# ChunLI-666/PointCloudProcessor

Hardware: AMD Instinct MI355X
Metric: Mpoints×frames/sec colorized (higher is better)
Workload: dtype f32/f64

## Files before the change

include/pcp_hip.h:

```cpp
#ifndef PCP_HIP_H
#define PCP_HIP_H

#include <stdint.h>

#ifdef __cplusplus
extern "C" {
#endif

#define PCP_ABI_VERSION 6

#define PCP_OK 0
#define PCP_ERR_INVALID (-1)
#define PCP_ERR_STATE (-2)
#define PCP_ERR_DEVICE (-3)
#define PCP_ERR_NOMEM (-4)
#define PCP_ERR_RANGE (-5)

typedef struct pcp_context pcp_context;

typedef struct pcp_pose {
  double x, y, z, qw, qx, qy, qz;
} pcp_pose;

typedef struct pcp_camera {
// ... 356 lines not shown
} pcp_cyl_frame;
int pcp_ortho_begin_cyl(pcp_context *ctx, const pcp_cyl_frame *frame);
int pcp_ortho_cyl_host(const pcp_cyl_frame *frame, int64_t n, const float *xyz, const uint8_t *rgb, const uint8_t *label,
                       const uint8_t *has, int64_t index_base, int32_t fill_radius_px, uint32_t *out_index, float *out_depth,
                       uint8_t *out_rgb, uint8_t *out_label, uint8_t *out_status, int32_t *out_source, int64_t *out_contributors,
                       int64_t *out_occupied, int64_t *out_filled);
int pcp_cyl_angle_host(int64_t n, const double *s, const double *t, double *out_theta);
int pcp_cyl_fit_host(int64_t n, const float *xyz, const float *normal, const uint8_t *has, const double *viewer, float gsd,
                     pcp_cyl_frame *out, double out_stats[8]);
int pcp_ortho_texture_cyl(pcp_context *ctx, const pcp_ortho_texture_params *params, uint8_t *out_rgb, uint8_t *out_mask,
                          uint8_t *out_status, int16_t *out_view, uint8_t *out_count, int64_t out_counts[4]);
int pcp_ortho_texture_points_cyl_host(const pcp_cyl_frame *frame, const pcp_ortho_texture_params *params, const int32_t *source,
                                      const float *depth, float *out_xyz, uint8_t *out_ok);
int pcp_cyl_sincos_host(int64_t n, const double *theta, double *out_sin, double *out_cos);

int pcp_close_pairs(pcp_context *ctx, double radius, int64_t *points_with_close_neighbour);

int pcp_timing_enable(pcp_context *ctx, int32_t on);
int pcp_timing_reset(pcp_context *ctx);
int pcp_timing_get(pcp_context *ctx, int32_t kernel_id, double *total_ms, int64_t *launches);
const char *pcp_kernel_name(int32_t kernel_id);
int pcp_tile_mask_density(pcp_context *ctx, double *kept_fraction);
int pcp_tile_masks(pcp_context *ctx, int64_t *tiles, int32_t *mask_words, uint32_t *out_words);
int pcp_cloud_order(pcp_context *ctx, int32_t *out_perm);
int pcp_tile_bounds(pcp_context *ctx, int64_t *tiles, float *out8);
int pcp_sor_redo_fraction(pcp_context *ctx, double *fraction);
int pcp_sor_distances(pcp_context *ctx, int64_t capacity, float *out_distance);
int pcp_selftest_arithmetic(pcp_context *ctx, int64_t samples, uint64_t seed, int64_t *mismatches_fp64,
                            int64_t *mismatches_fp32);
int pcp_selftest_visit_forms(pcp_context *ctx, int64_t samples, uint64_t seed, int64_t *mismatches_uv, int64_t *mismatches_cell,
                             int64_t *mismatches_sqrt, int32_t *short_distortion);
int pcp_selftest_k3_term(pcp_context *ctx, int64_t samples, uint64_t seed, int64_t *mismatches, int32_t *term_dropped);

#ifdef __cplusplus
}
#endif
#endif
```

pointcloudprocessor_amd/_build.py:

```python
from __future__ import annotations

import os
import subprocess

_PKG = os.path.dirname(os.path.abspath(__file__))
_ROOT = os.path.dirname(_PKG)
CSRC = os.path.join(_PKG, "csrc")
LIB_DIR = os.path.join(_PKG, "lib")
LIB_PATH = os.path.join(LIB_DIR, "libpcp_hip.so")
INCLUDE = os.path.join(_ROOT, "include")

SOURCES = ["pcp_context.hip", "pcp_colour.hip", "pcp_mls.hip", "pcp_grid.hip", "pcp_nid.hip", "pcp_hpr.hip", "pcp_colour_smooth.hip", "pcp_match.hip", "pcp_jpeg.hip",
           "pcp_stream_colour.hip", "pcp_ascii.hip", "pcp_ascii_parse.hip", "pcp_exposure.hip", "pcp_voxel_reduce.hip", "pcp_normals.hip", "pcp_mask_edt.hip", "pcp_ortho.hip", "pcp_ortho_texture.hip", "pcp_facets.hip", "pcp_crack_width.hip", "pcp_crack_fuse.hip", "pcp_crack_length.hip", "pcp_crack_skeleton.hip", "pcp_image_balance.hip"]
HEADERS = ["pcp_internal.hpp", "pcp_device.hpp", "pcp_scan.hpp", "pcp_hsv.hpp", "pcp_exact.hpp", "pcp_ascii.hpp", "pcp_ascii_parse.hpp", "pcp_visit_forms.hpp", "pcp_voxel_reduce.hpp", "pcp_eigen33.hpp", "pcp_eigen33_host.hpp", "pcp_facets.hpp", "pcp_normals.hpp", "pcp_mask_edt.hpp", "pcp_ortho.hpp", "pcp_ortho_cyl.hpp", "pcp_ortho_texture.hpp", "pcp_tile_classify.hpp", "pcp_tile_box.hpp", "pcp_crack_width.hpp", "pcp_crack_fuse.hpp", "pcp_crack_length.hpp", "pcp_crack_skeleton.hpp", "pcp_crack_map.hpp", "pcp_image_balance.hpp"]

HIPCC_FLAGS = [
    "--offload-arch=gfx950",
    "-O3",
    "-std=c++17",
    "-fPIC",
    "-ffp-contract=off",
    "-fhip-fp32-correctly-rounded-divide-sqrt",
    "-Wall",
    "-Wextra",
]


def _hipcc() -> str:
    for cand in (os.environ.get("HIPCC"), "/opt/rocm/bin/hipcc", "hipcc"):
        if cand and (os.path.isabs(cand) and os.path.exists(cand) or not os.path.isabs(cand)):
            return cand
    return "hipcc"


def source_sha256() -> str:
    import hashlib

# ... 57 lines not shown
```

pointcloudprocessor_amd/capi.py:

```python
from __future__ import annotations

import ctypes as C
import os
import re

import numpy as np

from . import _build

PCP_OK = 0
PCP_ERR_INVALID = -1
PCP_ERR_STATE = -2
PCP_ERR_DEVICE = -3
PCP_ERR_NOMEM = -4
PCP_ERR_RANGE = -5

NID_EVAL_FN = C.CFUNCTYPE(C.c_int, C.c_void_p, C.POINTER(C.c_double), C.c_int32, C.POINTER(C.c_double), C.POINTER(C.c_double),
                          C.POINTER(C.c_int32))
K_PROJECT, K_DEPTH, K_COLOUR, K_VISIBILITY, K_MLS_GRID, K_MLS_FIT, K_MISC, K_SOR, K_MLS_VOXEL, K_TILE_MASK, K_NID, K_HPR = range(12)
K_COLOUR_SMOOTH = 12
K_COUNT = 13


class PcpError(RuntimeError):
# ... 1648 lines not shown
    def selftest_arithmetic(self, samples: int = 1 << 26, seed: int = 1):
        a, b = C.c_int64(), C.c_int64()
        self._check(self.lib.pcp_selftest_arithmetic(self.h, C.c_int64(samples), C.c_uint64(seed), C.byref(a), C.byref(b)))
        return a.value, b.value

    def selftest_visit_forms(self, samples: int = 1 << 24, seed: int = 1):
        a, b, c, f = C.c_int64(), C.c_int64(), C.c_int64(), C.c_int32()
        self._check(self.lib.pcp_selftest_visit_forms(self.h, C.c_int64(samples), C.c_uint64(seed), C.byref(a), C.byref(b), C.byref(c),
                                                      C.byref(f)))
        return a.value, b.value, c.value, bool(f.value)

    def selftest_k3_term(self, samples: int = 1 << 24, seed: int = 1):
        a, f = C.c_int64(), C.c_int32()
        self._check(self.lib.pcp_selftest_k3_term(self.h, C.c_int64(samples), C.c_uint64(seed), C.byref(a), C.byref(f)))
        return a.value, bool(f.value)

    def tile_masks(self) -> np.ndarray:
        t, w = C.c_int64(), C.c_int32()
        self._check(self.lib.pcp_tile_masks(self.h, C.byref(t), C.byref(w), None))
        out = np.empty((t.value, w.value), np.uint32)
        self._check(self.lib.pcp_tile_masks(self.h, None, None, _ptr(out)))
        return out

    def cloud_order(self) -> np.ndarray:
        out = np.empty(int(self.lib.pcp_cloud_size(self.h)), np.int32)
        self._check(self.lib.pcp_cloud_order(self.h, _ptr(out)))
        return out

    def tile_bounds(self) -> tuple[np.ndarray, np.ndarray]:
        t = C.c_int64()
        self._check(self.lib.pcp_tile_bounds(self.h, C.byref(t), None))
        groups = (t.value + 15) // 16
        out = np.empty((t.value + groups, 8), np.float32)
        self._check(self.lib.pcp_tile_bounds(self.h, None, _ptr(out)))
        return out[:t.value], out[t.value:]

    def kernel_name(self, kernel_id: int) -> str:
        return self.lib.pcp_kernel_name(C.c_int32(kernel_id)).decode()
```

pointcloudprocessor_amd/csrc/pcp_colour.hip:

```cpp
#include <algorithm>
#include <cfloat>
#include <cstdlib>

#include "pcp_device.hpp"
#include "pcp_hsv.hpp"
#include "pcp_scan.hpp"
#include "pcp_tile_classify.hpp"

namespace pcp {

constexpr int kBlock = 256;
constexpr uint32_t kFltMaxBits = 0x7f7fffffu;

template <bool kCommon>
__device__ __forceinline__ DevCamera common_camera(const DevCamera &in) {
  DevCamera c = in;
  if constexpr (kCommon) {
    c.cull_mode = PCP_CULL_ZBUFFER;
    c.enable_zbuf = 1;
    c.pretest = 1;
    c.ds_fast = 1;
  }
  return c;
}
inline bool is_common_camera(const pcp_context *ctx) {
  const DevCamera &c = ctx->dcam;
  return c.cull_mode == PCP_CULL_ZBUFFER && c.enable_zbuf == 1 && c.pretest == 1 && c.ds_fast == 1 && ctx->uv_tame;
}

struct ProjectOut {
// ... 48 lines not shown
    if (out.pixel) *reinterpret_cast<int4 *>(out.pixel + i0) = pixel;
    if (out.xc) {
      *reinterpret_cast<float4 *>(out.xc + i0) = xc;
      *reinterpret_cast<float4 *>(out.yc + i0) = yc;
      *reinterpret_cast<float4 *>(out.zc + i0) = zc;
    }
  } else {
    for (int64_t i = i0; i < n; ++i) {
      int32_t cell, pixel;
      float range, xc, yc, zc;
      project_store_one(cam, fr, x[i], y[i], z[i], cell, pixel, range, xc, yc, zc);
      if (out.cell) out.cell[i] = cell;
      if (out.range) out.range[i] = range;
      if (out.pixel) out.pixel[i] = pixel;
      if (out.xc) {
        out.xc[i] = xc;
        out.yc[i] = yc;
        out.zc[i] = zc;
      }
    }
  }
}

constexpr int kTileGroup = 16;

__global__ __launch_bounds__(kBlock) void k_group_mask_flat(const float4 *__restrict__ bounds, int64_t groups, DevCamera cam,
                                                            const DevFrame *__restrict__ frames, int32_t n_frames,
                                                            int32_t w0, int32_t w1, int32_t words,
                                                            uint32_t *__restrict__ group_mask,
                                                            uint32_t *__restrict__ group_inside, int32_t cull_enabled,
                                                            int32_t *__restrict__ zeroed, int32_t n_zeroed,
                                                            unsigned long long *__restrict__ far_maps, int64_t far_cells) {
  const int64_t idx = static_cast<int64_t>(blockIdx.x) * kBlock + threadIdx.x;
  if (idx < n_zeroed) zeroed[idx] = 0;
  for (int64_t c = idx; c < far_cells; c += static_cast<int64_t>(gridDim.x) * kBlock) far_maps[c] = 0x7f7f7f7f7f7f7f7full;
  const int32_t nw = w1 - w0;
  const int64_t gw = idx >> 5;
  const int64_t group = gw / nw;
  const bool live = group < groups;
  const int32_t w = w0 + static_cast<int32_t>(gw - group * nw);
  const int32_t f = (w << 5) + static_cast<int32_t>(idx & 31);
  int cls = 1;
  if (live && f < n_frames) cls = cull_enabled ? tile_classify_box(cam, frames[f], bounds[2 * group], bounds[2 * group + 1]) : 0;
  const unsigned long long m = __ballot(cls != 1), in = __ballot(cls == 2);
  if (live && (idx & 31) == 0) {
    group_mask[group * words + w] = static_cast<uint32_t>((threadIdx.x & 32) ? (m >> 32) : m);
    group_inside[group * words + w] = static_cast<uint32_t>((threadIdx.x & 32) ? (in >> 32) : in);
  }
}

template <bool kInside>
__global__ __launch_bounds__(kBlock) void k_tile_mask_dense(const float4 *__restrict__ bounds, int64_t tiles,
                                                            DevCamera cam, const DevFrame *__restrict__ frames,
                                                            int32_t n_frames, int32_t w0, int32_t w1, int32_t words,
                                                            const uint32_t *__restrict__ group_mask,
                                                            const uint32_t *__restrict__ group_inside,
                                                            uint32_t *__restrict__ tile_mask,
                                                            uint32_t *__restrict__ inside_mask, int32_t cull_enabled) {
  const int lane = threadIdx.x & 63;
  const int32_t nw = w1 - w0;
  const int64_t gw = static_cast<int64_t>(blockIdx.x) * (kBlock / 64) + (threadIdx.x >> 6);
  const int64_t group = gw / nw;
  if (group >= (tiles + kTileGroup - 1) / kTileGroup) return;
  const int32_t w = w0 + static_cast<int32_t>(gw - group * nw);
  const int t = lane & 15, slot = lane >> 4;
  const int64_t tile = group * kTileGroup + t;
  const bool have = tile < tiles;
  uint32_t todo = __builtin_amdgcn_readfirstlane(group_mask[group * words + w]);
  const int32_t nb = n_frames - (w << 5);
  if (nb < 32) todo &= nb <= 0 ? 0u : ((1u << nb) - 1u);
// ... 1576 lines not shown
  if (rc != PCP_OK) return rc;
  if (frame_begin < 0 || frame_end > ctx->n_frames || frame_begin > frame_end)
    return set_error(ctx, PCP_ERR_RANGE, "pcp_depth_pass: keyframe range [%d,%d) outside 0..%d", frame_begin, frame_end,
                     ctx->n_frames);
  if (frame_begin == frame_end) return PCP_OK;
  if ((rc = ensure_depth(ctx)) != PCP_OK) return rc;
  const int64_t cells = cells_of(ctx);
  const int64_t map_cells = static_cast<int64_t>(frame_end - frame_begin) * cells;
  const bool z_maps = ctx->n > 0 && ctx->dcam.enable_zbuf;
  if (z_maps) {
    PCP_HIP_TRY(ctx, ctx->depth_sq.ensure(static_cast<size_t>(map_cells) + 4));
  } else if ((rc = fill_u32(ctx, ctx->depth.p + static_cast<int64_t>(frame_begin) * cells, map_cells, kFltMaxBits)) != PCP_OK) {
    return rc;
  }
  if (ctx->n > 0) {
    const size_t plane = plane_of(ctx);
    const int32_t w0 = frame_begin >> 5, w1 = ((frame_end - 1) >> 5) + 1;
    static const bool cull_tiles = [] {
      const char *e = std::getenv("PCP_DISABLE_TILE_CULL");
      return !(e && e[0] == '1');
    }();
    {
      LaunchTimer t(ctx, PCP_K_TILE_MASK);
      const int64_t groups = div_up(ctx->n_tiles, kTileGroup);
      const float4 *tile_bnd = reinterpret_cast<const float4 *>(ctx->tile_bounds.p);
      const size_t gwords = static_cast<size_t>(groups) * ctx->mask_words;
      PCP_HIP_TRY(ctx, ctx->group_mask.ensure(2 * gwords + 8));
      uint32_t *group_inside = ctx->group_mask.p + gwords + 4;
      hipLaunchKernelGGL(k_group_mask_flat, dim3(std::max(blocks_for(groups * (w1 - w0) * 32), blocks_for(2 * kWorkBins))),
                         dim3(kBlock), 0, ctx->stream, tile_bnd + 2 * ctx->n_tiles, groups, ctx->dcam, ctx->frames.p, ctx->n_frames,
                         w0, w1, ctx->mask_words, ctx->group_mask.p, group_inside, cull_tiles ? 1 : 0, ctx->work_hist.p,
                         2 * kWorkBins, z_maps ? reinterpret_cast<unsigned long long *>(ctx->depth_sq.p) : nullptr,
                         z_maps ? map_cells : int64_t(0));
      uint32_t *tile_inside = is_common_camera(ctx) ? nullptr : ctx->tile_inside.p;
      hipLaunchKernelGGL(tile_inside ? k_tile_mask_dense<true> : k_tile_mask_dense<false>, dim3(static_cast<uint32_t>(div_up(groups * (w1 - w0), kBlock / 64))), dim3(kBlock),
                         0, ctx->stream, tile_bnd, ctx->n_tiles, ctx->dcam, ctx->frames.p, ctx->n_frames, w0, w1,
                         ctx->mask_words, ctx->group_mask.p, group_inside, ctx->tile_mask.p, tile_inside, cull_tiles ? 1 : 0);
      if ((rc = sort_tiles_by_work(ctx, w0, w1, ctx->tile_order.p)) != PCP_OK) return rc;
      ctx->tile_order_live = true;
    }
    if (ctx->cull.cull_mode == PCP_CULL_HPR) {
      int rch = ensure_hull_bits(ctx);
      if (rch != PCP_OK) return rch;
      if (!ctx->depth_from_batch) {
        int32_t clear_until = frame_begin;
        for (int32_t f = frame_begin; f < frame_end; ++f) {
          uint32_t *hull_plane = ctx->hull_bits.p + static_cast<size_t>(f >> 5) * static_cast<size_t>(ctx->n);
          if ((f & 31) == 0 && std::min(f + 32, ctx->n_frames) <= frame_end) {
            PCP_HIP_TRY(ctx, hipMemsetAsync(hull_plane, 0, static_cast<size_t>(ctx->n) * 4, ctx->stream));
            clear_until = std::min(f + 32, ctx->n_frames);
          }
          if (f >= clear_until) {
            LaunchTimer t(ctx, PCP_K_HPR);
            hipLaunchKernelGGL(k_hull_clear, dim3(blocks_for(ctx->n)), dim3(kBlock), 0, ctx->stream, hull_plane, ctx->n, 1u << (f & 31));
// ... 388 lines not shown
  std::vector<uint32_t> h(static_cast<size_t>(ctx->n_tiles) * ctx->mask_words);
  PCP_HIP_TRY(ctx, hipMemcpyAsync(h.data(), ctx->tile_mask.p, h.size() * 4, hipMemcpyDeviceToHost, ctx->stream));
  PCP_HIP_TRY(ctx, hipStreamSynchronize(ctx->stream));
  uint64_t bits = 0;
  for (uint32_t w : h) bits += static_cast<uint64_t>(__builtin_popcount(w));
  *kept_fraction = static_cast<double>(bits) / (static_cast<double>(ctx->n_tiles) * ctx->n_frames);
  return PCP_OK;
}

int pcp_tile_masks(pcp_context *ctx, int64_t *tiles, int32_t *mask_words, uint32_t *out_words) {
  if (!ctx) return PCP_ERR_INVALID;
  if (!ctx->tile_mask.p || ctx->n_tiles == 0 || ctx->n_frames == 0)
    return set_error(ctx, PCP_ERR_STATE, "pcp_tile_masks: no masks (call pcp_depth_pass)");
  if (tiles) *tiles = ctx->n_tiles;
  if (mask_words) *mask_words = ctx->mask_words;
  if (out_words) {
    PCP_HIP_TRY(ctx, hipMemcpyAsync(out_words, ctx->tile_mask.p, static_cast<size_t>(ctx->n_tiles) * ctx->mask_words * 4,
                                    hipMemcpyDeviceToHost, ctx->stream));
    PCP_HIP_TRY(ctx, hipStreamSynchronize(ctx->stream));
  }
  return PCP_OK;
}

int pcp_cloud_order(pcp_context *ctx, int32_t *out_perm) {
  if (!ctx || !out_perm) return PCP_ERR_INVALID;
  if (ctx->n == 0) return set_error(ctx, PCP_ERR_STATE, "pcp_cloud_order: no cloud (call pcp_upload_cloud)");
  PCP_HIP_TRY(ctx, hipMemcpyAsync(out_perm, ctx->perm.p, static_cast<size_t>(ctx->n) * 4, hipMemcpyDeviceToHost, ctx->stream));
  PCP_HIP_TRY(ctx, hipStreamSynchronize(ctx->stream));
  return PCP_OK;
}

int pcp_tile_bounds(pcp_context *ctx, int64_t *tiles, float *out8) {
  if (!ctx) return PCP_ERR_INVALID;
  if (ctx->n == 0 || ctx->n_tiles == 0 || !ctx->tile_bounds.p)
    return set_error(ctx, PCP_ERR_STATE, "pcp_tile_bounds: no cloud (call pcp_upload_cloud)");
  if (tiles) *tiles = ctx->n_tiles;
  if (out8) {
    const int64_t groups = div_up(ctx->n_tiles, kTileGroup);
    PCP_HIP_TRY(ctx, hipMemcpyAsync(out8, ctx->tile_bounds.p, static_cast<size_t>(ctx->n_tiles + groups) * 8 * 4, hipMemcpyDeviceToHost,
                                    ctx->stream));
    PCP_HIP_TRY(ctx, hipStreamSynchronize(ctx->stream));
  }
  return PCP_OK;
}

int pcp_colour_result_device(pcp_context *ctx, void **device_ptr, int64_t *n_words) {
// ... 114 lines not shown
```

pointcloudprocessor_amd/csrc/pcp_context.hip:

```cpp
#include <algorithm>
#include <cfloat>
#include <cmath>
#include <cstdlib>
#include <new>
#include <vector>

#include "pcp_internal.hpp"
#include "pcp_crack_map.hpp"
#include "pcp_visit_forms.hpp"
#include "pcp_scan.hpp"

namespace pcp {

static thread_local std::string g_error;

int set_error(const pcp_context *ctx, int code, const char *fmt, ...) {
  char buf[1024];
  va_list ap;
  va_start(ap, fmt);
  vsnprintf(buf, sizeof(buf), fmt, ap);
  va_end(ap);
  if (ctx)
    ctx->error = buf;
  else
    g_error = buf;
  return code;
}

void set_global_error(const char *fmt, ...) {
  char buf[1024];
  va_list ap;
  va_start(ap, fmt);
  vsnprintf(buf, sizeof(buf), fmt, ap);
// ... 254 lines not shown
                                                       int64_t n, float *__restrict__ sx, float *__restrict__ sy,
                                                       float *__restrict__ sz, int32_t *__restrict__ inv_perm) {
  const int64_t j = static_cast<int64_t>(blockIdx.x) * kUpBlock + threadIdx.x;
  if (j >= n) return;
  const int32_t i = perm[j];
  sx[j] = x[i];
  sy[j] = y[i];
  sz[j] = z[i];
  if (inv_perm) inv_perm[i] = static_cast<int32_t>(j);
}

template <int kSpan>
__global__ __launch_bounds__(kUpBlock) void k_up_bounds(const float *__restrict__ sx, const float *__restrict__ sy,
                                                        const float *__restrict__ sz, int64_t n,
                                                        float4 *__restrict__ out, int64_t count) {
  constexpr int kLanes = kSpan >= kUpBlock ? kUpBlock : kSpan;
  constexpr int kPer = kSpan / kLanes;
  constexpr int kSpheresPerBlock = kUpBlock / kLanes;
  __shared__ double red[10][kUpBlock / 64];
  const int sub = threadIdx.x / kLanes, l = threadIdx.x % kLanes;
  const int64_t sphere = static_cast<int64_t>(blockIdx.x) * kSpheresPerBlock + sub;
  const int64_t b = sphere * kSpan;
  double lo[3] = {1e300, 1e300, 1e300}, hi[3] = {-1e300, -1e300, -1e300};
  float px[kPer], py[kPer], pz[kPer];
  bool have[kPer];
#pragma unroll
  for (int q = 0; q < kPer; ++q) {
    const int64_t j = b + static_cast<int64_t>(q) * kLanes + l;
    have[q] = sphere < count && j < n;
    px[q] = have[q] ? sx[j] : 0.0f;
    py[q] = have[q] ? sy[j] : 0.0f;
    pz[q] = have[q] ? sz[j] : 0.0f;
    if (have[q]) {
      lo[0] = fmin(lo[0], static_cast<double>(px[q])); hi[0] = fmax(hi[0], static_cast<double>(px[q]));
      lo[1] = fmin(lo[1], static_cast<double>(py[q])); hi[1] = fmax(hi[1], static_cast<double>(py[q]));
      lo[2] = fmin(lo[2], static_cast<double>(pz[q])); hi[2] = fmax(hi[2], static_cast<double>(pz[q]));
    }
  }
#pragma unroll
  for (int a = 0; a < 3; ++a)
    for (int o = (kLanes < 64 ? kLanes : 64) / 2; o >= 1; o >>= 1) {
      lo[a] = fmin(lo[a], __shfl_xor(lo[a], o, 64));
      hi[a] = fmax(hi[a], __shfl_xor(hi[a], o, 64));
    }
  if (kLanes > 64) {
    if ((threadIdx.x & 63) == 0)
      for (int a = 0; a < 3; ++a) {
        red[a][threadIdx.x >> 6] = lo[a];
        red[3 + a][threadIdx.x >> 6] = hi[a];
      }
    __syncthreads();
    for (int a = 0; a < 3; ++a)
      for (int k = 0; k < kUpBlock / 64; ++k) {
        lo[a] = fmin(lo[a], red[a][k]);
        hi[a] = fmax(hi[a], red[3 + a][k]);
      }
    __syncthreads();
  }
  float c[3];
#pragma unroll
  for (int a = 0; a < 3; ++a) c[a] = static_cast<float>(0.5 * (lo[a] + hi[a]));
  double r2 = 0.0, h[3] = {0.0, 0.0, 0.0};
#pragma unroll
  for (int q = 0; q < kPer; ++q)
    if (have[q]) {
      const double dx = static_cast<double>(px[q]) - static_cast<double>(c[0]);
      const double dy = static_cast<double>(py[q]) - static_cast<double>(c[1]);
      const double dz = static_cast<double>(pz[q]) - static_cast<double>(c[2]);
      r2 = fmax(r2, (dx * dx + dy * dy) + dz * dz);
      h[0] = fmax(h[0], fabs(dx));
      h[1] = fmax(h[1], fabs(dy));
      h[2] = fmax(h[2], fabs(dz));
    }
  for (int o = (kLanes < 64 ? kLanes : 64) / 2; o >= 1; o >>= 1) {
    r2 = fmax(r2, __shfl_xor(r2, o, 64));
#pragma unroll
    for (int a = 0; a < 3; ++a) h[a] = fmax(h[a], __shfl_xor(h[a], o, 64));
  }
  if (kLanes > 64) {
    if ((threadIdx.x & 63) == 0) {
      red[6][threadIdx.x >> 6] = r2;
      for (int a = 0; a < 3; ++a) red[7 + a][threadIdx.x >> 6] = h[a];
    }
    __syncthreads();
    for (int k = 0; k < kUpBlock / 64; ++k) {
      r2 = fmax(r2, red[6][k]);
      for (int a = 0; a < 3; ++a) h[a] = fmax(h[a], red[7 + a][k]);
    }
  }
  if (l == 0 && sphere < count) {
    const auto up = [](double v) {
      const float r = static_cast<float>(v * (1.0 + 1e-6));
      return isfinite(r) ? __uint_as_float(__float_as_uint(r) + 1u) : r;
    };
    out[2 * sphere] = make_float4(c[0], c[1], c[2], up(sqrt(r2)));
    out[2 * sphere + 1] = make_float4(up(h[0]), up(h[1]), up(h[2]), 0.0f);
// ... 117 lines not shown
    hipLaunchKernelGGL(k_up_deinterleave, dim3(up_blocks(n)), dim3(kUpBlock), 0, st, static_cast<const uint32_t *>(aos), stride / 4, n,
                       dx, dy, dz);
  } else if (aos) {
    PCP_HIP_TRY(ctx, raw.ensure(static_cast<size_t>(n) * static_cast<size_t>(stride) / 4 + 4));
    PCP_HIP_TRY(ctx, hipMemcpyAsync(raw.p, aos, static_cast<size_t>(n) * static_cast<size_t>(stride), hipMemcpyHostToDevice, st));
    hipLaunchKernelGGL(k_up_deinterleave, dim3(up_blocks(n)), dim3(kUpBlock), 0, st, raw.p, stride / 4, n, dx, dy, dz);
  } else {
    PCP_HIP_TRY(ctx, hipMemcpyAsync(dx, x, sn * 4, hipMemcpyHostToDevice, st));
    PCP_HIP_TRY(ctx, hipMemcpyAsync(dy, y, sn * 4, hipMemcpyHostToDevice, st));
    PCP_HIP_TRY(ctx, hipMemcpyAsync(dz, z, sn * 4, hipMemcpyHostToDevice, st));
  }
  float mn[3], mx[3];
  unsigned long long nonfinite = 0;
  PCP_HIP_TRY(ctx, ctx->inv_perm.ensure(plane + 4));
  if (int rc = spatial_order(ctx, dx, dy, dz, n, ctx->perm.p, ctx->sxyz.p, ctx->sxyz.p + plane, ctx->sxyz.p + 2 * plane,
                             ctx->inv_perm.p, mn, mx, &nonfinite))
    return rc;
  raw.release();
  ctx->nonfinite_points = static_cast<int64_t>(nonfinite);
  for (int a = 0; a < 3; ++a) {
    ctx->host_min[a] = mn[a];
    ctx->host_max[a] = mx[a];
  }
  const int64_t tiles = (n + 63) / 64, groups = (tiles + 15) / 16;
  PCP_HIP_TRY(ctx, ctx->tile_bounds.ensure(static_cast<size_t>(tiles + groups) * 8 + 4));
  float4 *sph = reinterpret_cast<float4 *>(ctx->tile_bounds.p);
  hipLaunchKernelGGL(k_up_bounds<64>, dim3(static_cast<uint32_t>((tiles + 3) / 4)), dim3(kUpBlock), 0, st, ctx->sxyz.p,
                     ctx->sxyz.p + plane, ctx->sxyz.p + 2 * plane, n, sph, tiles);
  hipLaunchKernelGGL(k_up_bounds<1024>, dim3(static_cast<uint32_t>(groups)), dim3(kUpBlock), 0, st, ctx->sxyz.p,
                     ctx->sxyz.p + plane, ctx->sxyz.p + 2 * plane, n, sph + 2 * tiles, groups);
  PCP_HIP_TRY(ctx, hipGetLastError());
  ctx->n_tiles = tiles;
  PCP_HIP_TRY(ctx, hipStreamSynchronize(st));
  return PCP_OK;
}

}

using namespace pcp;

extern "C" {

int pcp_abi_version(void) { return PCP_ABI_VERSION; }

int pcp_create(int32_t device, pcp_context **out) {
  if (!out) {
    set_global_error("pcp_create: out is NULL");
    return PCP_ERR_INVALID;
  }
  *out = nullptr;
  int count = 0;
  hipError_t e = hipGetDeviceCount(&count);
  if (e != hipSuccess || count <= 0) {
// ... 408 lines not shown
```

pointcloudprocessor_amd/host_build.py:

```python
from __future__ import annotations

import os
import subprocess

from . import _build

HOST = os.path.join(os.path.dirname(os.path.abspath(__file__)), "host")
BIN = os.path.join(HOST, "bin")
ROCM = os.environ.get("ROCM_PATH", "/opt/rocm")

TARGETS = {
    "pcp_shim_selftest": ["shim_selftest.cpp"],
    "PointCloudProcessor": ["main.cpp"],
    "image_dump": ["image_dump.cpp"],
    "format_selftest": ["format_selftest.cpp"],
    "parse_selftest": ["parse_selftest.cpp"],
    "visit_forms_selftest": ["visit_forms_selftest.cpp"],
    "k3_term_selftest": ["k3_term_selftest.cpp"],
    "voxel_reduce_selftest": ["voxel_reduce_selftest.cpp"],
    "normals_selftest": ["normals_selftest.cpp"],
    "ortho_selftest": ["ortho_selftest.cpp"],
    "ortho_texture_selftest": ["ortho_texture_selftest.cpp"],
    "crack_width_selftest": ["crack_width_selftest.cpp"],
    "crack_fuse_selftest": ["crack_fuse_selftest.cpp"],
    "crack_length_selftest": ["crack_length_selftest.cpp"],
    "crack_skeleton_selftest": ["crack_skeleton_selftest.cpp"],
    "image_balance_selftest": ["image_balance_selftest.cpp"],
    "ortho_cyl_selftest": ["ortho_cyl_selftest.cpp"],
    "ortho_cyl_texture_selftest": ["ortho_cyl_texture_selftest.cpp"],
    "facets_selftest": ["facets_selftest.cpp"],
    "tile_bounds_selftest": ["tile_bounds_selftest.cpp"],
}


def build(force: bool = False) -> dict:
    os.makedirs(BIN, exist_ok=True)
    out = {}
    for name, srcs in TARGETS.items():
        exe = os.path.join(BIN, name)
        deps = [os.path.join(HOST, s) for s in srcs] + [os.path.join(HOST, "pcp_shim.hpp"), os.path.join(HOST, "pcp_multi.hpp"), os.path.join(HOST, "pcd_io.hpp"), os.path.join(HOST, "image_io.hpp"), os.path.join(HOST, "pcd_device_reader.hpp"),
                                                       os.path.join(_build.CSRC, "pcp_ascii_parse.hpp"), os.path.join(_build.CSRC, "pcp_ascii.hpp"), os.path.join(_build.CSRC, "pcp_visit_forms.hpp"), os.path.join(_build.CSRC, "pcp_voxel_reduce.hpp"), os.path.join(_build.CSRC, "pcp_normals.hpp"), os.path.join(_build.CSRC, "pcp_ortho.hpp"), os.path.join(_build.CSRC, "pcp_ortho_cyl.hpp"), os.path.join(_build.CSRC, "pcp_ortho_texture.hpp"), os.path.join(_build.CSRC, "pcp_crack_width.hpp"), os.path.join(_build.CSRC, "pcp_crack_fuse.hpp"), os.path.join(_build.CSRC, "pcp_crack_length.hpp"), os.path.join(_build.CSRC, "pcp_crack_skeleton.hpp"), os.path.join(_build.CSRC, "pcp_image_balance.hpp"), os.path.join(_build.CSRC, "pcp_hsv.hpp"), os.path.join(_build.CSRC, "pcp_facets.hpp"), os.path.join(_build.CSRC, "pcp_eigen33_host.hpp"), os.path.join(_build.CSRC, "pcp_tile_box.hpp"),
                                                       os.path.join(_build.INCLUDE, "pcp_hip.h")]
        deps = [d for d in deps if os.path.exists(d)]
        stale = force or not os.path.exists(exe) or any(os.path.getmtime(d) > os.path.getmtime(exe) for d in deps)
        if stale:
            extra = os.environ.get("PCP_HOST_CXXFLAGS", "").split()
            multi = ["-D__HIP_PLATFORM_AMD__", "-isystem", os.path.join(ROCM, "include")] if name == "PointCloudProcessor" else []
            multi_libs = ["-L", os.path.join(ROCM, "lib"), "-lrccl", "-lamdhip64", "-Wl,-rpath," + os.path.join(ROCM, "lib")] \
                if name == "PointCloudProcessor" else []
            cmd = ["g++", "-std=c++17", "-O2", "-ffp-contract=off", "-pthread", "-Wall", "-Wextra"] + extra + multi + ["-I", _build.INCLUDE, "-I", HOST] + [
                os.path.join(HOST, s) for s in srcs] + ["-L", _build.LIB_DIR, "-lpcp_hip"] + multi_libs + [
                                                        "-lz", "-Wl,-rpath,$ORIGIN/../../lib", "-o", exe]
            proc = subprocess.run(cmd, capture_output=True, text=True)
            if proc.returncode != 0:
                raise RuntimeError(f"g++ failed for {name}:\n{proc.stderr[-3000:]}")
        out[name] = exe
    return out
```

Measured before the change: 2.079 million.

## Cull tile groups top-down through a new block level of bounding boxes

Result: no change. 2.078 million (-0.1%).

```diff
diff --git a/include/pcp_hip.h b/include/pcp_hip.h
--- a/include/pcp_hip.h
+++ b/include/pcp_hip.h
@@ -402,6 +402,7 @@
 const char *pcp_kernel_name(int32_t kernel_id);
 int pcp_tile_mask_density(pcp_context *ctx, double *kept_fraction);
 int pcp_tile_masks(pcp_context *ctx, int64_t *tiles, int32_t *mask_words, uint32_t *out_words);
+int pcp_tile_work(pcp_context *ctx, int64_t *tiles, int32_t *out_work);
 int pcp_cloud_order(pcp_context *ctx, int32_t *out_perm);
 int pcp_tile_bounds(pcp_context *ctx, int64_t *tiles, float *out8);
 int pcp_sor_redo_fraction(pcp_context *ctx, double *fraction);
diff --git a/pointcloudprocessor_amd/_build.py b/pointcloudprocessor_amd/_build.py
--- a/pointcloudprocessor_amd/_build.py
+++ b/pointcloudprocessor_amd/_build.py
@@ -12,7 +12,7 @@
 
 SOURCES = ["pcp_context.hip", "pcp_colour.hip", "pcp_mls.hip", "pcp_grid.hip", "pcp_nid.hip", "pcp_hpr.hip", "pcp_colour_smooth.hip", "pcp_match.hip", "pcp_jpeg.hip",
            "pcp_stream_colour.hip", "pcp_ascii.hip", "pcp_ascii_parse.hip", "pcp_exposure.hip", "pcp_voxel_reduce.hip", "pcp_normals.hip", "pcp_mask_edt.hip", "pcp_ortho.hip", "pcp_ortho_texture.hip", "pcp_facets.hip", "pcp_crack_width.hip", "pcp_crack_fuse.hip", "pcp_crack_length.hip", "pcp_crack_skeleton.hip", "pcp_image_balance.hip"]
-HEADERS = ["pcp_internal.hpp", "pcp_device.hpp", "pcp_scan.hpp", "pcp_hsv.hpp", "pcp_exact.hpp", "pcp_ascii.hpp", "pcp_ascii_parse.hpp", "pcp_visit_forms.hpp", "pcp_voxel_reduce.hpp", "pcp_eigen33.hpp", "pcp_eigen33_host.hpp", "pcp_facets.hpp", "pcp_normals.hpp", "pcp_mask_edt.hpp", "pcp_ortho.hpp", "pcp_ortho_cyl.hpp", "pcp_ortho_texture.hpp", "pcp_tile_classify.hpp", "pcp_tile_box.hpp", "pcp_crack_width.hpp", "pcp_crack_fuse.hpp", "pcp_crack_length.hpp", "pcp_crack_skeleton.hpp", "pcp_crack_map.hpp", "pcp_image_balance.hpp"]
+HEADERS = ["pcp_internal.hpp", "pcp_device.hpp", "pcp_scan.hpp", "pcp_hsv.hpp", "pcp_exact.hpp", "pcp_ascii.hpp", "pcp_ascii_parse.hpp", "pcp_visit_forms.hpp", "pcp_voxel_reduce.hpp", "pcp_eigen33.hpp", "pcp_eigen33_host.hpp", "pcp_facets.hpp", "pcp_normals.hpp", "pcp_mask_edt.hpp", "pcp_ortho.hpp", "pcp_ortho_cyl.hpp", "pcp_ortho_texture.hpp", "pcp_tile_classify.hpp", "pcp_tile_box.hpp", "pcp_tile_levels.hpp", "pcp_crack_width.hpp", "pcp_crack_fuse.hpp", "pcp_crack_length.hpp", "pcp_crack_skeleton.hpp", "pcp_crack_map.hpp", "pcp_image_balance.hpp"]
 
 HIPCC_FLAGS = [
     "--offload-arch=gfx950",
diff --git a/pointcloudprocessor_amd/capi.py b/pointcloudprocessor_amd/capi.py
--- a/pointcloudprocessor_amd/capi.py
+++ b/pointcloudprocessor_amd/capi.py
@@ -1694,6 +1694,13 @@
         self._check(self.lib.pcp_tile_masks(self.h, None, None, _ptr(out)))
         return out
 
+    def tile_work(self) -> np.ndarray:
+        t = C.c_int64()
+        self._check(self.lib.pcp_tile_work(self.h, C.byref(t), None))
+        out = np.empty(t.value, np.int32)
+        self._check(self.lib.pcp_tile_work(self.h, None, _ptr(out)))
+        return out
+
     def cloud_order(self) -> np.ndarray:
         out = np.empty(int(self.lib.pcp_cloud_size(self.h)), np.int32)
         self._check(self.lib.pcp_cloud_order(self.h, _ptr(out)))
diff --git a/pointcloudprocessor_amd/csrc/pcp_colour.hip b/pointcloudprocessor_amd/csrc/pcp_colour.hip
--- a/pointcloudprocessor_amd/csrc/pcp_colour.hip
+++ b/pointcloudprocessor_amd/csrc/pcp_colour.hip
@@ -6,6 +6,7 @@
 #include "pcp_hsv.hpp"
 #include "pcp_scan.hpp"
 #include "pcp_tile_classify.hpp"
+#include "pcp_tile_levels.hpp"
 
 namespace pcp {
 
@@ -100,30 +101,59 @@
   }
 }
 
-constexpr int kTileGroup = 16;
-
-__global__ __launch_bounds__(kBlock) void k_group_mask_flat(const float4 *__restrict__ bounds, int64_t groups, DevCamera cam,
-                                                            const DevFrame *__restrict__ frames, int32_t n_frames,
-                                                            int32_t w0, int32_t w1, int32_t words,
-                                                            uint32_t *__restrict__ group_mask,
-                                                            uint32_t *__restrict__ group_inside, int32_t cull_enabled,
-                                                            int32_t *__restrict__ zeroed, int32_t n_zeroed,
-                                                            unsigned long long *__restrict__ far_maps, int64_t far_cells) {
+constexpr int kTileGroup = kGroupTiles;
+
+__global__ __launch_bounds__(kBlock) void k_group_mask_top_down(const float4 *__restrict__ bounds,
+                                                                const float4 *__restrict__ block_bounds, int64_t groups,
+                                                                int64_t blocks, DevCamera cam,
+                                                                const DevFrame *__restrict__ frames, int32_t n_frames,
+                                                                int32_t w0, int32_t w1, int32_t words,
+                                                                uint32_t *__restrict__ group_mask,
+                                                                uint32_t *__restrict__ group_inside, int32_t cull_enabled,
+                                                                int32_t *__restrict__ zeroed, int32_t n_zeroed,
+                                                                unsigned long long *__restrict__ far_maps, int64_t far_cells) {
+  __shared__ uint32_t s_keep[kBlockGroups][kSpanWords], s_in[kBlockGroups][kSpanWords];
+  __shared__ int32_t s_list[64];
+  __shared__ int32_t s_count;
   const int64_t idx = static_cast<int64_t>(blockIdx.x) * kBlock + threadIdx.x;
   if (idx < n_zeroed) zeroed[idx] = 0;
   for (int64_t c = idx; c < far_cells; c += static_cast<int64_t>(gridDim.x) * kBlock) far_maps[c] = 0x7f7f7f7f7f7f7f7full;
-  const int32_t nw = w1 - w0;
-  const int64_t gw = idx >> 5;
-  const int64_t group = gw / nw;
-  const bool live = group < groups;
-  const int32_t w = w0 + static_cast<int32_t>(gw - group * nw);
-  const int32_t f = (w << 5) + static_cast<int32_t>(idx & 31);
-  int cls = 1;
-  if (live && f < n_frames) cls = cull_enabled ? tile_classify_box(cam, frames[f], bounds[2 * group], bounds[2 * group + 1]) : 0;
-  const unsigned long long m = __ballot(cls != 1), in = __ballot(cls == 2);
-  if (live && (idx & 31) == 0) {
-    group_mask[group * words + w] = static_cast<uint32_t>((threadIdx.x & 32) ? (m >> 32) : m);
-    group_inside[group * words + w] = static_cast<uint32_t>((threadIdx.x & 32) ? (in >> 32) : in);
+  const int32_t spans = mask_spans(w0, w1);
+  const int64_t blk = blockIdx.x / spans;
+  if (blk >= blocks) return;
+  const int32_t wb = w0 + (static_cast<int32_t>(blockIdx.x - blk * spans)) * kSpanWords;
+  const int32_t ng = block_group_count(blk, groups);
+  const int64_t g0 = block_first_group(blk);
+  if (threadIdx.x < 64) {
+    const int32_t lane = threadIdx.x;
+    const int32_t f = (wb << 5) + lane;
+    int cls = 1;
+    if (wb + (lane >> 5) < w1 && f < n_frames)
+      cls = cull_enabled ? tile_classify_box(cam, frames[f], block_bounds[2 * blk], block_bounds[2 * blk + 1]) : 0;
+    const unsigned long long in = __ballot(cls == 2), open = __ballot(cls == 0);
+    if (lane < kBlockGroups * kSpanWords)
+      s_keep[lane / kSpanWords][lane % kSpanWords] = s_in[lane / kSpanWords][lane % kSpanWords] =
+          static_cast<uint32_t>(in >> (32 * (lane % kSpanWords)));
+    if (cls == 0) s_list[__popcll(open & ((1ull << lane) - 1ull))] = lane;
+    if (lane == 0) s_count = __popcll(open);
+  }
+  __syncthreads();
+  const int32_t pairs = s_count * kBlockGroups;
+  for (int32_t p = threadIdx.x; p < pairs; p += kBlock) {
+    const int32_t g = p % kBlockGroups, k = s_list[p / kBlockGroups];
+    if (g < ng) {
+      const int cls = cull_enabled ? tile_classify_box(cam, frames[(wb << 5) + k], bounds[2 * (g0 + g)], bounds[2 * (g0 + g) + 1]) : 0;
+      if (cls != 1) atomicOr(&s_keep[g][k >> 5], 1u << (k & 31));
+      if (cls == 2) atomicOr(&s_in[g][k >> 5], 1u << (k & 31));
+    }
+  }
+  __syncthreads();
+  if (threadIdx.x < kBlockGroups * kSpanWords) {
+    const int32_t g = threadIdx.x / kSpanWords, w = wb + threadIdx.x % kSpanWords;
+    if (g < ng && w < w1) {
+      group_mask[(g0 + g) * words + w] = s_keep[g][threadIdx.x % kSpanWords];
+      group_inside[(g0 + g) * words + w] = s_in[g][threadIdx.x % kSpanWords];
+    }
   }
 }
 
@@ -1746,14 +1776,16 @@
     }();
     {
       LaunchTimer t(ctx, PCP_K_TILE_MASK);
-      const int64_t groups = div_up(ctx->n_tiles, kTileGroup);
+      const TileLevels lv = tile_levels(ctx->n);
+      const int64_t groups = lv.groups;
       const float4 *tile_bnd = reinterpret_cast<const float4 *>(ctx->tile_bounds.p);
       const size_t gwords = static_cast<size_t>(groups) * ctx->mask_words;
       PCP_HIP_TRY(ctx, ctx->group_mask.ensure(2 * gwords + 8));
       uint32_t *group_inside = ctx->group_mask.p + gwords + 4;
-      hipLaunchKernelGGL(k_group_mask_flat, dim3(std::max(blocks_for(groups * (w1 - w0) * 32), blocks_for(2 * kWorkBins))),
-                         dim3(kBlock), 0, ctx->stream, tile_bnd + 2 * ctx->n_tiles, groups, ctx->dcam, ctx->frames.p, ctx->n_frames,
-                         w0, w1, ctx->mask_words, ctx->group_mask.p, group_inside, cull_tiles ? 1 : 0, ctx->work_hist.p,
+      hipLaunchKernelGGL(k_group_mask_top_down,
+                         dim3(std::max(static_cast<uint32_t>(lv.blocks * mask_spans(w0, w1)), blocks_for(2 * kWorkBins))), dim3(kBlock), 0,
+                         ctx->stream, tile_bnd + 2 * lv.group_at, tile_bnd + 2 * lv.block_at, groups, lv.blocks, ctx->dcam, ctx->frames.p,
+                         ctx->n_frames, w0, w1, ctx->mask_words, ctx->group_mask.p, group_inside, cull_tiles ? 1 : 0, ctx->work_hist.p,
                          2 * kWorkBins, z_maps ? reinterpret_cast<unsigned long long *>(ctx->depth_sq.p) : nullptr,
                          z_maps ? map_cells : int64_t(0));
       uint32_t *tile_inside = is_common_camera(ctx) ? nullptr : ctx->tile_inside.p;
@@ -2188,6 +2220,18 @@
   return PCP_OK;
 }
 
+int pcp_tile_work(pcp_context *ctx, int64_t *tiles, int32_t *out_work) {
+  if (!ctx) return PCP_ERR_INVALID;
+  if (!ctx->tile_work.p || !ctx->tile_order_live || ctx->n_tiles == 0)
+    return set_error(ctx, PCP_ERR_STATE, "pcp_tile_work: no tile order (call pcp_depth_pass)");
+  if (tiles) *tiles = ctx->n_tiles;
+  if (out_work) {
+    PCP_HIP_TRY(ctx, hipMemcpyAsync(out_work, ctx->tile_work.p, static_cast<size_t>(ctx->n_tiles) * 4, hipMemcpyDeviceToHost, ctx->stream));
+    PCP_HIP_TRY(ctx, hipStreamSynchronize(ctx->stream));
+  }
+  return PCP_OK;
+}
+
 int pcp_cloud_order(pcp_context *ctx, int32_t *out_perm) {
   if (!ctx || !out_perm) return PCP_ERR_INVALID;
   if (ctx->n == 0) return set_error(ctx, PCP_ERR_STATE, "pcp_cloud_order: no cloud (call pcp_upload_cloud)");
diff --git a/pointcloudprocessor_amd/csrc/pcp_context.hip b/pointcloudprocessor_amd/csrc/pcp_context.hip
--- a/pointcloudprocessor_amd/csrc/pcp_context.hip
+++ b/pointcloudprocessor_amd/csrc/pcp_context.hip
@@ -9,6 +9,7 @@
 #include "pcp_crack_map.hpp"
 #include "pcp_visit_forms.hpp"
 #include "pcp_scan.hpp"
+#include "pcp_tile_levels.hpp"
 
 namespace pcp {
 
@@ -309,19 +310,33 @@
   const int64_t sphere = static_cast<int64_t>(blockIdx.x) * kSpheresPerBlock + sub;
   const int64_t b = sphere * kSpan;
   double lo[3] = {1e300, 1e300, 1e300}, hi[3] = {-1e300, -1e300, -1e300};
-  float px[kPer], py[kPer], pz[kPer];
-  bool have[kPer];
+  constexpr bool kKeep = kPer <= 4;
+  constexpr int kKept = kKeep ? kPer : 1;
+  float px[kKept], py[kKept], pz[kKept];
+  bool have[kKept];
+  if constexpr (kKeep) {
 #pragma unroll
-  for (int q = 0; q < kPer; ++q) {
-    const int64_t j = b + static_cast<int64_t>(q) * kLanes + l;
-    have[q] = sphere < count && j < n;
-    px[q] = have[q] ? sx[j] : 0.0f;
-    py[q] = have[q] ? sy[j] : 0.0f;
-    pz[q] = have[q] ? sz[j] : 0.0f;
-    if (have[q]) {
-      lo[0] = fmin(lo[0], static_cast<double>(px[q])); hi[0] = fmax(hi[0], static_cast<double>(px[q]));
-      lo[1] = fmin(lo[1], static_cast<double>(py[q])); hi[1] = fmax(hi[1], static_cast<double>(py[q]));
-      lo[2] = fmin(lo[2], static_cast<double>(pz[q])); hi[2] = fmax(hi[2], static_cast<double>(pz[q]));
+    for (int q = 0; q < kPer; ++q) {
+      const int64_t j = b + static_cast<int64_t>(q) * kLanes + l;
+      have[q] = sphere < count && j < n;
+      px[q] = have[q] ? sx[j] : 0.0f;
+      py[q] = have[q] ? sy[j] : 0.0f;
+      pz[q] = have[q] ? sz[j] : 0.0f;
+      if (have[q]) {
+        lo[0] = fmin(lo[0], static_cast<double>(px[q])); hi[0] = fmax(hi[0], static_cast<double>(px[q]));
+        lo[1] = fmin(lo[1], static_cast<double>(py[q])); hi[1] = fmax(hi[1], static_cast<double>(py[q]));
+        lo[2] = fmin(lo[2], static_cast<double>(pz[q])); hi[2] = fmax(hi[2], static_cast<double>(pz[q]));
+      }
+    }
+  } else {
+    for (int q = 0; q < kPer; ++q) {
+      const int64_t j = b + static_cast<int64_t>(q) * kLanes + l;
+      if (sphere < count && j < n) {
+        const double vx = sx[j], vy = sy[j], vz = sz[j];
+        lo[0] = fmin(lo[0], vx); hi[0] = fmax(hi[0], vx);
+        lo[1] = fmin(lo[1], vy); hi[1] = fmax(hi[1], vy);
+        lo[2] = fmin(lo[2], vz); hi[2] = fmax(hi[2], vz);
+      }
     }
   }
 #pragma unroll
@@ -348,17 +363,25 @@
 #pragma unroll
   for (int a = 0; a < 3; ++a) c[a] = static_cast<float>(0.5 * (lo[a] + hi[a]));
   double r2 = 0.0, h[3] = {0.0, 0.0, 0.0};
+  const auto member = [&](float mx, float my, float mz) {
+    const double dx = static_cast<double>(mx) - static_cast<double>(c[0]);
+    const double dy = static_cast<double>(my) - static_cast<double>(c[1]);
+    const double dz = static_cast<double>(mz) - static_cast<double>(c[2]);
+    r2 = fmax(r2, (dx * dx + dy * dy) + dz * dz);
+    h[0] = fmax(h[0], fabs(dx));
+    h[1] = fmax(h[1], fabs(dy));
+    h[2] = fmax(h[2], fabs(dz));
+  };
+  if constexpr (kKeep) {
 #pragma unroll
-  for (int q = 0; q < kPer; ++q)
-    if (have[q]) {
-      const double dx = static_cast<double>(px[q]) - static_cast<double>(c[0]);
-      const double dy = static_cast<double>(py[q]) - static_cast<double>(c[1]);
-      const double dz = static_cast<double>(pz[q]) - static_cast<double>(c[2]);
-      r2 = fmax(r2, (dx * dx + dy * dy) + dz * dz);
-      h[0] = fmax(h[0], fabs(dx));
-      h[1] = fmax(h[1], fabs(dy));
-      h[2] = fmax(h[2], fabs(dz));
-    }
+    for (int q = 0; q < kPer; ++q)
+      if (have[q]) member(px[q], py[q], pz[q]);
+  } else {
+    for (int q = 0; q < kPer; ++q) {
+      const int64_t j = b + static_cast<int64_t>(q) * kLanes + l;
+      if (sphere < count && j < n) member(sx[j], sy[j], sz[j]);
+    }
+  }
   for (int o = (kLanes < 64 ? kLanes : 64) / 2; o >= 1; o >>= 1) {
     r2 = fmax(r2, __shfl_xor(r2, o, 64));
 #pragma unroll
@@ -522,13 +545,16 @@
     ctx->host_min[a] = mn[a];
     ctx->host_max[a] = mx[a];
   }
-  const int64_t tiles = (n + 63) / 64, groups = (tiles + 15) / 16;
-  PCP_HIP_TRY(ctx, ctx->tile_bounds.ensure(static_cast<size_t>(tiles + groups) * 8 + 4));
+  const TileLevels lv = tile_levels(n);
+  const int64_t tiles = lv.tiles, groups = lv.groups;
+  PCP_HIP_TRY(ctx, ctx->tile_bounds.ensure(static_cast<size_t>(lv.records) * 8 + 4));
   float4 *sph = reinterpret_cast<float4 *>(ctx->tile_bounds.p);
-  hipLaunchKernelGGL(k_up_bounds<64>, dim3(static_cast<uint32_t>((tiles + 3) / 4)), dim3(kUpBlock), 0, st, ctx->sxyz.p,
+  hipLaunchKernelGGL(k_up_bounds<kTilePlaces>, dim3(static_cast<uint32_t>((tiles + 3) / 4)), dim3(kUpBlock), 0, st, ctx->sxyz.p,
                      ctx->sxyz.p + plane, ctx->sxyz.p + 2 * plane, n, sph, tiles);
-  hipLaunchKernelGGL(k_up_bounds<1024>, dim3(static_cast<uint32_t>(groups)), dim3(kUpBlock), 0, st, ctx->sxyz.p,
-                     ctx->sxyz.p + plane, ctx->sxyz.p + 2 * plane, n, sph + 2 * tiles, groups);
+  hipLaunchKernelGGL(k_up_bounds<kGroupPlaces>, dim3(static_cast<uint32_t>(groups)), dim3(kUpBlock), 0, st, ctx->sxyz.p,
+                     ctx->sxyz.p + plane, ctx->sxyz.p + 2 * plane, n, sph + 2 * lv.group_at, groups);
+  hipLaunchKernelGGL(k_up_bounds<kBlockPlaces>, dim3(static_cast<uint32_t>(lv.blocks)), dim3(kUpBlock), 0, st, ctx->sxyz.p,
+                     ctx->sxyz.p + plane, ctx->sxyz.p + 2 * plane, n, sph + 2 * lv.block_at, lv.blocks);
   PCP_HIP_TRY(ctx, hipGetLastError());
   ctx->n_tiles = tiles;
   PCP_HIP_TRY(ctx, hipStreamSynchronize(st));
diff --git a/pointcloudprocessor_amd/csrc/pcp_tile_levels.hpp b/pointcloudprocessor_amd/csrc/pcp_tile_levels.hpp
--- /dev/null
+++ b/pointcloudprocessor_amd/csrc/pcp_tile_levels.hpp
@@ -0,0 +1,46 @@
+#pragma once
+
+#include <cstdint>
+
+#if defined(__HIPCC__)
+#include <hip/hip_runtime.h>
+#define PCP_TL_HD __host__ __device__ __forceinline__
+#else
+#define PCP_TL_HD inline
+#endif
+
+namespace pcp {
+
+constexpr int kTilePlaces = 64;
+constexpr int kGroupTiles = 16;
+constexpr int kBlockGroups = 16;
+constexpr int kGroupPlaces = kTilePlaces * kGroupTiles;
+constexpr int kBlockPlaces = kGroupPlaces * kBlockGroups;
+
+struct TileLevels {
+  int64_t tiles, groups, blocks;
+  int64_t group_at, block_at;
+  int64_t records;
+};
+
+PCP_TL_HD TileLevels tile_levels(int64_t n) {
+  TileLevels t;
+  t.tiles = (n + kTilePlaces - 1) / kTilePlaces;
+  t.groups = (t.tiles + kGroupTiles - 1) / kGroupTiles;
+  t.blocks = (t.groups + kBlockGroups - 1) / kBlockGroups;
+  t.group_at = t.tiles;
+  t.block_at = t.tiles + t.groups;
+  t.records = t.tiles + t.groups + t.blocks;
+  return t;
+}
+
+PCP_TL_HD int64_t block_first_group(int64_t b) { return b * kBlockGroups; }
+PCP_TL_HD int32_t block_group_count(int64_t b, int64_t groups) {
+  const int64_t left = groups - b * kBlockGroups;
+  return static_cast<int32_t>(left < 0 ? 0 : left > kBlockGroups ? kBlockGroups : left);
+}
+
+constexpr int kSpanWords = 2;
+PCP_TL_HD int32_t mask_spans(int32_t w0, int32_t w1) { return (w1 - w0 + kSpanWords - 1) / kSpanWords; }
+
+}
diff --git a/pointcloudprocessor_amd/host/tile_levels_selftest.cpp b/pointcloudprocessor_amd/host/tile_levels_selftest.cpp
--- /dev/null
+++ b/pointcloudprocessor_amd/host/tile_levels_selftest.cpp
@@ -0,0 +1,90 @@
+#include <cstdint>
+#include <cstdio>
+#include <cstdlib>
+#include <vector>
+
+#include "../csrc/pcp_tile_levels.hpp"
+
+static long failures = 0;
+#define CHECK(cond)                                                        \
+  do {                                                                     \
+    if (!(cond)) {                                                         \
+      if (++failures < 20) std::printf("FAILED line %d: %s\n", __LINE__, #cond); \
+    }                                                                      \
+  } while (0)
+
+static std::vector<int32_t> tile_places, group_tiles, block_groups;
+static void add_place(int64_t j) {
+  const size_t t = static_cast<size_t>(j / 64);
+  if (t >= tile_places.size()) {
+    tile_places.push_back(0);
+    const size_t g = t / 16;
+    if (g >= group_tiles.size()) {
+      group_tiles.push_back(0);
+      const size_t b = g / 16;
+      if (b >= block_groups.size()) block_groups.push_back(0);
+      ++block_groups[b];
+    }
+    ++group_tiles[g];
+  }
+  ++tile_places[t];
+}
+static void check_by_walking(int64_t n) {
+  if (n > 0) add_place(n - 1);
+  const pcp::TileLevels lv = pcp::tile_levels(n);
+  CHECK(lv.tiles == static_cast<int64_t>(tile_places.size()));
+  CHECK(lv.groups == static_cast<int64_t>(group_tiles.size()));
+  CHECK(lv.blocks == static_cast<int64_t>(block_groups.size()));
+  CHECK(lv.group_at == lv.tiles && lv.block_at == lv.tiles + lv.groups && lv.records == lv.block_at + lv.blocks);
+  int64_t seen = 0;
+  for (int64_t b = 0; b < lv.blocks; ++b) {
+    CHECK(pcp::block_first_group(b) == seen);
+    CHECK(pcp::block_group_count(b, lv.groups) == block_groups[static_cast<size_t>(b)]);
+    seen += pcp::block_group_count(b, lv.groups);
+  }
+  CHECK(seen == lv.groups);
+  CHECK(pcp::block_group_count(lv.blocks, lv.groups) == 0 && pcp::block_group_count(lv.blocks + 5, lv.groups) == 0);
+}
+
+static void check_large(int64_t n) {
+  const pcp::TileLevels lv = pcp::tile_levels(n);
+  CHECK(lv.tiles * 64 >= n && (lv.tiles - 1) * 64 < n);
+  CHECK(lv.groups * 16 >= lv.tiles && (lv.groups - 1) * 16 < lv.tiles);
+  CHECK(lv.blocks * 16 >= lv.groups && (lv.blocks - 1) * 16 < lv.groups);
+  CHECK(lv.records == lv.tiles + lv.groups + lv.blocks);
+  int64_t seen = 0;
+  for (int64_t b = 0; b < lv.blocks; ++b) {
+    const int32_t c = pcp::block_group_count(b, lv.groups);
+    CHECK(c >= 1 && c <= 16 && (c == 16 || b == lv.blocks - 1));
+    seen += c;
+  }
+  CHECK(seen == lv.groups);
+}
+
+static void check_spans() {
+  for (int32_t w0 = 0; w0 < 70; ++w0)
+    for (int32_t w1 = w0 + 1; w1 < 140; ++w1) {
+      std::vector<int> hit(static_cast<size_t>(w1), 0);
+      const int32_t spans = pcp::mask_spans(w0, w1);
+      for (int32_t s = 0; s < spans; ++s)
+        for (int k = 0; k < pcp::kSpanWords; ++k) {
+          const int32_t w = w0 + s * pcp::kSpanWords + k;
+          if (w < w1) ++hit[static_cast<size_t>(w)];
+        }
+      for (int32_t w = 0; w < w1; ++w) CHECK(hit[static_cast<size_t>(w)] == (w >= w0 ? 1 : 0));
+    }
+}
+
+int main(int argc, char **argv) {
+  const int64_t limit = argc > 1 ? std::atoll(argv[1]) : 70000;
+  static_assert(pcp::kGroupPlaces == 1024 && pcp::kBlockPlaces == 16384, "level spans");
+  for (int64_t n = 0; n <= limit; ++n) check_by_walking(n);
+  const int64_t edges[] = {65535, 65536, 65537, 16384 * 16 - 1, 16384 * 16, 16384 * 16 + 1, 10000000, (int64_t(1) << 31) - 1,
+                           int64_t(1) << 31, (int64_t(1) << 31) + 1, (int64_t(1) << 32) + 12345};
+  for (int64_t n : edges) check_large(n);
+  check_spans();
+  std::printf("tile levels: sizes 0 ... %ld walked, %zu large sizes, word ranges up to 140 words\n", static_cast<long>(limit),
+              sizeof(edges) / sizeof(edges[0]));
+  std::printf("tile_levels_selftest: %ld failures\n", failures);
+  return failures ? 1 : 0;
+}
diff --git a/pointcloudprocessor_amd/host_build.py b/pointcloudprocessor_amd/host_build.py
--- a/pointcloudprocessor_amd/host_build.py
+++ b/pointcloudprocessor_amd/host_build.py
@@ -30,6 +30,7 @@
     "ortho_cyl_texture_selftest": ["ortho_cyl_texture_selftest.cpp"],
     "facets_selftest": ["facets_selftest.cpp"],
     "tile_bounds_selftest": ["tile_bounds_selftest.cpp"],
+    "tile_levels_selftest": ["tile_levels_selftest.cpp"],
 }
 
 
@@ -39,7 +40,7 @@
     for name, srcs in TARGETS.items():
         exe = os.path.join(BIN, name)
         deps = [os.path.join(HOST, s) for s in srcs] + [os.path.join(HOST, "pcp_shim.hpp"), os.path.join(HOST, "pcp_multi.hpp"), os.path.join(HOST, "pcd_io.hpp"), os.path.join(HOST, "image_io.hpp"), os.path.join(HOST, "pcd_device_reader.hpp"),
-                                                       os.path.join(_build.CSRC, "pcp_ascii_parse.hpp"), os.path.join(_build.CSRC, "pcp_ascii.hpp"), os.path.join(_build.CSRC, "pcp_visit_forms.hpp"), os.path.join(_build.CSRC, "pcp_voxel_reduce.hpp"), os.path.join(_build.CSRC, "pcp_normals.hpp"), os.path.join(_build.CSRC, "pcp_ortho.hpp"), os.path.join(_build.CSRC, "pcp_ortho_cyl.hpp"), os.path.join(_build.CSRC, "pcp_ortho_texture.hpp"), os.path.join(_build.CSRC, "pcp_crack_width.hpp"), os.path.join(_build.CSRC, "pcp_crack_fuse.hpp"), os.path.join(_build.CSRC, "pcp_crack_length.hpp"), os.path.join(_build.CSRC, "pcp_crack_skeleton.hpp"), os.path.join(_build.CSRC, "pcp_image_balance.hpp"), os.path.join(_build.CSRC, "pcp_hsv.hpp"), os.path.join(_build.CSRC, "pcp_facets.hpp"), os.path.join(_build.CSRC, "pcp_eigen33_host.hpp"), os.path.join(_build.CSRC, "pcp_tile_box.hpp"),
+                                                       os.path.join(_build.CSRC, "pcp_ascii_parse.hpp"), os.path.join(_build.CSRC, "pcp_ascii.hpp"), os.path.join(_build.CSRC, "pcp_visit_forms.hpp"), os.path.join(_build.CSRC, "pcp_voxel_reduce.hpp"), os.path.join(_build.CSRC, "pcp_normals.hpp"), os.path.join(_build.CSRC, "pcp_ortho.hpp"), os.path.join(_build.CSRC, "pcp_ortho_cyl.hpp"), os.path.join(_build.CSRC, "pcp_ortho_texture.hpp"), os.path.join(_build.CSRC, "pcp_crack_width.hpp"), os.path.join(_build.CSRC, "pcp_crack_fuse.hpp"), os.path.join(_build.CSRC, "pcp_crack_length.hpp"), os.path.join(_build.CSRC, "pcp_crack_skeleton.hpp"), os.path.join(_build.CSRC, "pcp_image_balance.hpp"), os.path.join(_build.CSRC, "pcp_hsv.hpp"), os.path.join(_build.CSRC, "pcp_facets.hpp"), os.path.join(_build.CSRC, "pcp_eigen33_host.hpp"), os.path.join(_build.CSRC, "pcp_tile_box.hpp"), os.path.join(_build.CSRC, "pcp_tile_levels.hpp"),
                                                        os.path.join(_build.INCLUDE, "pcp_hip.h")]
         deps = [d for d in deps if os.path.exists(d)]
         stale = force or not os.path.exists(exe) or any(os.path.getmtime(d) > os.path.getmtime(exe) for d in deps)
diff --git a/profiles/listing_compare.py b/profiles/listing_compare.py
--- /dev/null
+++ b/profiles/listing_compare.py
@@ -0,0 +1,64 @@
+#!/usr/bin/env python3
+import re
+import subprocess
+import sys
+
+
+def demangle(names):
+    try:
+        out = subprocess.run(["c++filt"], input="\n".join(names), capture_output=True, text=True, check=True).stdout.split("\n")
+        return dict(zip(names, out))
+    except (OSError, subprocess.CalledProcessError):
+        return {n: n for n in names}
+
+
+def functions(path):
+    funcs, regs, cur, body = {}, {}, None, []
+    for line in open(path):
+        m = re.match(r"^(\w+):\s*(;.*)?$", line)
+        if m and not m.group(1).startswith(".L") and cur is None and not line.startswith("\t"):
+            cur, body = m.group(1), []
+            continue
+        if cur is not None:
+            if re.match(r"^\.Lfunc_end\d+:", line):
+                labels = {}
+                text = []
+                for ins in body:
+                    ins = re.sub(r"\.LBB\d+_\d+", lambda k: labels.setdefault(k.group(0), f"L{len(labels)}"), ins)
+                    text.append(ins)
+                funcs[cur] = text
+                cur = None
+                continue
+            s = line.split(";")[0].strip()
+            if not s or s.startswith(".") and not s.startswith(".LBB"):
+                continue
+            body.append(s)
+        m = re.match(r"^; (\w+Gprs|NumSgprs|NumVgprs|ScratchSize|Occupancy): (\d+)", line)
+        if m and funcs:
+            regs.setdefault(list(funcs)[-1], {})[m.group(1)] = int(m.group(2))
+    return funcs, regs
+
+
+def main():
+    a, ra = functions(sys.argv[1])
+    b, rb = functions(sys.argv[2])
+    names = demangle(sorted(set(a) | set(b)))
+    same = [n for n in a if n in b and a[n] == b[n]]
+    diff = [n for n in a if n in b and a[n] != b[n]]
+    print(f"{len(a)} functions in the parent, {len(b)} in the tree; {len(same)} equal instruction for instruction")
+    for n in diff:
+        print("differs:", names[n], len(a[n]), "->", len(b[n]), "instructions", ra.get(n), rb.get(n))
+    for n in a:
+        if n not in b:
+            print("only in the parent:", names[n], len(a[n]), "instructions", ra.get(n))
+    for n in b:
+        if n not in a:
+            print("only in the tree:", names[n], len(b[n]), "instructions", rb.get(n))
+    for want in sys.argv[3:]:
+        for n in b:
+            if want in names[n]:
+                print(names[n], len(b[n]), "instructions", rb.get(n), "(tree)", "| parent:", len(a[n]) if n in a else None, ra.get(n))
+
+
+if __name__ == "__main__":
+    main()
diff --git a/profiles/mask_stage_probe.py b/profiles/mask_stage_probe.py
--- /dev/null
+++ b/profiles/mask_stage_probe.py
@@ -0,0 +1,37 @@
+#!/usr/bin/env python3
+import json
+import os
+import sys
+import time
+
+import numpy as np
+
+sys.path.insert(0, os.path.dirname(os.path.dirname(os.path.abspath(__file__))))
+import torch
+
+from pointcloudprocessor_amd import capi, synth
+
+WARM = int(sys.argv[1]) if len(sys.argv) > 1 else 300
+STEPS = int(sys.argv[2]) if len(sys.argv) > 2 else 40
+cam = synth.camera_dict("cfg")
+N, F = 10_000_000, 256
+x, y, z, _ = synth.make_cloud(N)
+poses, _ = synth.make_trajectory(F)
+ctx = capi.Context(0)
+ctx.set_camera(capi.camera_from_dict(cam))
+ctx.upload_cloud(x, y, z)
+ctx.set_frames(poses)
+imgs = [synth.make_image(f, cam["image_width"], cam["image_height"]) for f in range(8)]
+for f in range(F):
+    ctx.upload_image(f, imgs[f % 8])
+for _ in range(WARM):
+    ctx.colorize(download=False)
+ctx.synchronize()
+t = time.perf_counter()
+for _ in range(STEPS):
+    ctx.colorize(download=False)
+ctx.synchronize()
+step = (time.perf_counter() - t) / STEPS
+out = ctx.download_result_packed()
+print(json.dumps({"lib": os.environ.get("PCP_HIP_LIBRARY", "default"), "warm": WARM, "steps": STEPS, "step_ms": round(step * 1e3, 4),
+                  "coloured": int(((out >> 24) & 1).sum()), "checksum": int(out.astype(np.uint64).sum())}))
diff --git a/profiles/tile_rounds_sim.py b/profiles/tile_rounds_sim.py
--- /dev/null
+++ b/profiles/tile_rounds_sim.py
@@ -0,0 +1,45 @@
+#!/usr/bin/env python3
+import os
+import sys
+import time
+
+import numpy as np
+
+sys.path.insert(0, os.path.dirname(os.path.dirname(os.path.abspath(__file__))))
+sys.path.insert(0, os.path.dirname(os.path.abspath(__file__)))
+import tile_bounds_sim as sim
+from oracle import np_oracle
+from pointcloudprocessor_amd import synth
+
+
+def main():
+    n = int(sys.argv[1]) if len(sys.argv) > 1 else 10_000_000
+    F = sim.F_ALL
+    cam = synth.camera_dict("cfg")
+    ds = 14
+    mw, mh = cam["cull_width"] // ds, cam["cull_height"] // ds
+    box = (-(ds + 0.5), -(ds + 0.5), max(ds * mw, cam["image_width"]) + 0.5, max(ds * mh, cam["image_height"]) + 0.5)
+    x, y, z, _ = synth.make_cloud(n)
+    poses, _ = synth.make_trajectory(F)
+    t0 = time.time()
+    p = np.stack([x, y, z], axis=1)
+    p = p[sim.hilbert_order(p)]
+    gc, gr, gh = sim.bounds(p, 1024)
+    print(f"# {n} points, {len(gc)} groups, {F} keyframes; order and bounds in {time.time() - t0:.0f} s", flush=True)
+    todo = np.zeros((len(gc), F), bool)
+    for f in range(F):
+        todo[:, f] = sim.classify(cam, box, np_oracle.pose_to_matrices(poses[f])[0], gc, gr, gh) == 0
+    pairs = int(todo.sum())
+    print(f"open (group, keyframe) pairs {pairs / 1e6:.3f} M = {pairs * 16 / 1e6:.2f} M tile classifications")
+    print("| keyframes per wavefront | wavefronts with work | rounds | against 32 | mean fill of a round's four keyframe slots |")
+    print("|---|---|---|---|---|")
+    base = None
+    for span in (32, 64, 128, 256):
+        c = todo.reshape(len(gc), F // span, span).sum(axis=2)
+        rounds = int(((c + 3) // 4).sum())
+        base = base or rounds
+        print(f"| {span} | {int((c > 0).sum())} | {rounds} | {100 * (rounds / base - 1):+.1f} % | {pairs / (4 * rounds):.3f} |")
+
+
+if __name__ == "__main__":
+    main()
```
